# CogSP/CoEvoNet

Hardware: AMD Instinct MI355X
Metric: env-steps/sec (agent-steps of the whole job; generations/sec in gens_per_sec), Co-GA simple_adversary_v3 pop=200 HoF=5 (higher is better)
Workload: dtype f32

## Files before the change

### coevonet_amd/csrc/fc_forward.hip

```cpp
#include <cstdlib>

#include "coevo_common.hip.h"

namespace coevo {

#ifndef COEVO_HEAVY16_U
#define COEVO_HEAVY16_U 4
#endif
#ifndef COEVO_LIGHT_U
#define COEVO_LIGHT_U 8
#endif

typedef float f32x4_t __attribute__((ext_vector_type(4)));
__device__ inline float4 load_stream16(const float4 *p)
{
#ifdef COEVO_NO_NT
    return *p;
#else
    const f32x4_t v = __builtin_nontemporal_load(reinterpret_cast<const f32x4_t *>(p));
    return make_float4(v[0], v[1], v[2], v[3]);
#endif
}

template <int R, int P>
// ... 323 lines not shown
    if (row_wave && l < R * NACT) {
        const int r = l / NACT, o = l % NACT;
        float y = p_b3;
        const float4 *wr = reinterpret_cast<const float4 *>(&sm.w3s[pw][o][0]);
        const float4 *xr = reinterpret_cast<const float4 *>(&sm.h2[pw][r][0]);
#pragma unroll 8
        for (int k = 0; k < H2 / 4; ++k) {
            const float4 wv = wr[k], xv = xr[k];
            y = __builtin_fmaf(wv.x, xv.x, y);
            y = __builtin_fmaf(wv.y, xv.y, y);
            y = __builtin_fmaf(wv.z, xv.z, y);
            y = __builtin_fmaf(wv.w, xv.w, y);
        }
        sm.logit[pw][r][o] = y;
    }
    __syncthreads();
    COEVO_STAMP(5);

    if (row_wave && l < nrows[pw]) {
        int best = -1;
        float cur = -__builtin_inff();
#pragma unroll
        for (int o = 0; o < NACT; ++o) {
            const float v = sm.logit[pw][l][o];
            if (!__builtin_isfinite(v)) st |= COEVO_ST_BAD_OUT;
            if (v > cur) { cur = v; best = o; }
        }
        if (best < 0) { st |= COEVO_ST_NO_ACTION; best = 0; }
        const int row = row0[pw] + l;
        if constexpr (MODE >= MODE_FUSED) {
            a.act_cur[3 * a.row_game[row] + a.row_slot[row]] = best;
        } else {
            a.actions[row] = best;
        }
        if (a.logits) {
#pragma unroll
            for (int o = 0; o < NACT; ++o) a.logits[(size_t)row * COEVO_LOGIT_STRIDE + o] = sm.logit[pw][l][o];
        }
    }
    if (st) atomicOr(a.status, st);
    COEVO_STAMP(6);
}

template <int R>
struct FcSmemC {
    static constexpr int NG = (R + 3) / 4;
    static constexpr int RP = 4 * NG + 1;
    union {
        float par[13 * H1];
        float h1q[128][RP][4];
        float h1r[R][H1];
        struct { float h2[R][260]; float w3s[NACT][260]; } tail;
    };
    float xs0[4 * NG][COEVO_OBS_STRIDE];
    float red[4][16], red2[4][16];
    float logit[R][COEVO_LOGIT_STRIDE];
};

constexpr int FC2_MFMA = 0, FC2_DPP = 1;

#ifndef COEVO_SMALL_U
#define COEVO_SMALL_U 16
#endif

template <int J>
__device__ __forceinline__ void fmac_bcast(float &acc, float xv, float w)
{
    asm("v_fmac_f32_dpp %0, %1, %2 row_newbcast:%3 row_mask:0xf bank_mask:0xf" : "+v"(acc) : "v"(xv), "v"(w), "n"(J));
}

template <int R>
__device__ __forceinline__ void fmac_block16(float (&acc)[R], const float (&xv)[R], const float4 &p0, const float4 &p1,
                                             const float4 &p2, const float4 &p3)
{
#define COEVO_FMAC_K(J, W)                                   \
    _Pragma("unroll") for (int r = 0; r < R; ++r) fmac_bcast<J>(acc[r], xv[r], W);
    COEVO_FMAC_K(0, p0.x) COEVO_FMAC_K(1, p0.y) COEVO_FMAC_K(2, p0.z) COEVO_FMAC_K(3, p0.w)
    COEVO_FMAC_K(4, p1.x) COEVO_FMAC_K(5, p1.y) COEVO_FMAC_K(6, p1.z) COEVO_FMAC_K(7, p1.w)
    COEVO_FMAC_K(8, p2.x) COEVO_FMAC_K(9, p2.y) COEVO_FMAC_K(10, p2.z) COEVO_FMAC_K(11, p2.w)
    COEVO_FMAC_K(12, p3.x) COEVO_FMAC_K(13, p3.y) COEVO_FMAC_K(14, p3.z) COEVO_FMAC_K(15, p3.w)
#undef COEVO_FMAC_K
}

template <int R, int MODE, int FC2 = FC2_MFMA>
__device__ __forceinline__ void fc_policy_body_c(const FcArgs &a, FcSmemC<R> &sm, const coevo_fc_task *tasks, int first,
                                                 int n_tasks)
{
    static_assert((MODE == MODE_FUSED || MODE == MODE_OBS) && R * NACT <= 64 && R <= 8, "the lean merged cycle kernel");
    typedef float f32x4_acc __attribute__((ext_vector_type(4)));
    constexpr int NG = FcSmemC<R>::NG;
    COEVO_STAMP(0);
    const int t = threadIdx.x, w = t >> 6, l = t & 63;
    const bool active = first < n_tasks;
    const coevo_fc_task task = tasks[active ? first : n_tasks - 1];
    const int D = task.D, nrows = active ? task.n_rows : 0, row0 = task.row_begin;
    const float *net = a.slab + task.net_off;
    int st = 0;

    const int n_pieces = (D + 3) * (H1 / 4);
#pragma unroll
    for (int j = 0; j < 7; ++j)
        if (64 * w + 256 * j < n_pieces)
            __builtin_amdgcn_global_load_lds((const __attribute__((address_space(1))) void *)(net + 4 * (t + 256 * j)),
                                             (__attribute__((address_space(3))) void *)(&sm.par[4 * (64 * w + 256 * j)]),
                                             16, 0, 0);
    const float *b2p = net + fc_off_b2(D);
    float w3r[5];
    {
        const float *W3 = net + fc_off_w3(D);
#pragma unroll
        for (int j = 0; j < 5; ++j) w3r[j] = W3[t + 256 * j];
    }
    const float p_b2 = b2p[t], p_g2 = b2p[H2 + t], p_be2 = b2p[2 * H2 + t];
    const float p_b3 = (w == 0 && l < R * NACT) ? net[fc_off_b3(D) + l % NACT] : 0.0f;
    constexpr int US = COEVO_SMALL_U;
    static_assert(US % 4 == 0 && 128 % (2 * US) == 0, "buffers of whole 16-k blocks, consumed in pairs");
    const float4 *wps = reinterpret_cast<const float4 *>(net + fc_off_w2(D)) + (size_t)w * 128 * 64 + l;
    float4 sbufA[FC2 == FC2_DPP ? US : 1], sbufB[FC2 == FC2_DPP ? US : 1];

    if (w == 0 && l < 4 * NG) {
        float o[COEVO_OBS_STRIDE];
#pragma unroll
        for (int k = 0; k < COEVO_OBS_STRIDE; ++k) o[k] = 0.0f;
        if (l < nrows) {
            const int row = row0 + l;
            if constexpr (MODE == MODE_FUSED) {
                mpe_fused_observe(a.state, a.state_next, a.act_prev, a.game_limit, a.n_games, a.row_game[row],
                                  a.row_slot[row], a.cycle, a.pos_first, o);
            } else {
#pragma unroll
                for (int k = 0; k < 10; ++k) o[k] = (k < D) ? a.obs[(size_t)row * COEVO_OBS_STRIDE + k] : 0.0f;
            }
#pragma unroll
            for (int k = 0; k < 10; ++k)
                if (!__builtin_isfinite(o[k])) st |= COEVO_ST_BAD_INPUT;
        }
#pragma unroll
        for (int k = 0; k < COEVO_OBS_STRIDE; ++k) sm.xs0[l][k] = o[k];
    }
    COEVO_WSTAMP(0);
    __syncthreads();
    COEVO_WSTAMP(1);
    COEVO_CSTAMP(10);
    COEVO_STAMP(1);
    if constexpr (FC2 == FC2_DPP) {
#pragma unroll
        for (int uu = 0; uu < US; ++uu) sbufA[uu] = wps[(size_t)uu * 64];
#pragma unroll
        for (int uu = 0; uu < US; ++uu) sbufB[uu] = wps[(size_t)(US + uu) * 64];
    }

    const float *b1s = sm.par + D * H1;
    f32x4_acc c0[NG], c1[NG];
    {
        const float bia = b1s[t], bib = b1s[t + 256];
#pragma unroll
        for (int g = 0; g < NG; ++g)
#pragma unroll
            for (int i = 0; i < 4; ++i) { c0[g][i] = bia; c1[g][i] = bib; }
        float4 xk[NG][3];
#pragma unroll
        for (int g = 0; g < NG; ++g)
#pragma unroll
            for (int j = 0; j < 3; ++j) xk[g][j] = *reinterpret_cast<const float4 *>(&sm.xs0[4 * g + (l & 3)][4 * j]);
#pragma unroll
        for (int k = 0; k < 10; ++k) {
            if (k < D) {
                const float wa = sm.par[k * H1 + t], wb = sm.par[k * H1 + 256 + t];
#pragma unroll
                for (int g = 0; g < NG; ++g) {
// ... 4 lines not shown
                }
            }
        }
    }
    const float p_g1a = b1s[H1 + t], p_g1b = b1s[H1 + t + 256], p_be1a = b1s[2 * H1 + t], p_be1b = b1s[2 * H1 + t + 256];
    COEVO_STAMP(8);
    float v[2 * R];
#pragma unroll
    for (int r = 0; r < R; ++r) { v[2 * r] = c0[r >> 2][r & 3]; v[2 * r + 1] = c1[r >> 2][r & 3]; }
    {
        const float s = packed_totals<2 * R>(v, l);
        if (l < 2 * R) sm.red[w][l] = s;
    }
    COEVO_STAMP(9);
    COEVO_WSTAMP(2);
    __syncthreads();
    COEVO_WSTAMP(3);
    COEVO_STAMP(10);
    const int lr = l < R ? l : R - 1;
    {
        float tot = sm.red[0][2 * lr];
#pragma unroll
        for (int b = 1; b < 8; ++b) tot = tot + sm.red[b & 3][2 * lr + (b >> 2)];
        const float meanv = tot * (1.0f / H1);
#pragma unroll
        for (int r = 0; r < R; ++r) {
            const float m = __int_as_float(__builtin_amdgcn_readlane(__float_as_int(meanv), r));
            v[2 * r] = v[2 * r] - m;
            v[2 * r + 1] = v[2 * r + 1] - m;
        }
    }
    {
        float sq[2 * R];
#pragma unroll
        for (int j = 0; j < 2 * R; ++j) sq[j] = v[j] * v[j];
        const float s = packed_totals<2 * R>(sq, l);
        if (l < 2 * R) sm.red2[w][l] = s;
    }
    COEVO_WSTAMP(4);
    __syncthreads();
    COEVO_WSTAMP(5);
    {
        float tot = sm.red2[0][2 * lr];
#pragma unroll
        for (int b = 1; b < 8; ++b) tot = tot + sm.red2[b & 3][2 * lr + (b >> 2)];
        const float rstdv = 1.0f / __builtin_sqrtf(tot * (1.0f / H1) + LN_EPS);
        bool bad = false;
#pragma unroll
        for (int r = 0; r < R; ++r) {
            const float rstd = __int_as_float(__builtin_amdgcn_readlane(__float_as_int(rstdv), r));
            const float y0 = __builtin_fmaf(v[2 * r] * rstd, p_g1a, p_be1a);
            const float y1 = __builtin_fmaf(v[2 * r + 1] * rstd, p_g1b, p_be1b);
            if (r < nrows) bad = bad || bad_post_relu(y0) || bad_post_relu(y1);
            if constexpr (FC2 == FC2_DPP) {
                sm.h1r[r][t] = relu_keep_nan(y0);
                sm.h1r[r][t + 256] = relu_keep_nan(y1);
            } else {
                sm.h1q[t >> 2][r][t & 3] = relu_keep_nan(y0);
                sm.h1q[(t + 256) >> 2][r][t & 3] = relu_keep_nan(y1);
            }
        }
        if (bad) st |= COEVO_ST_BAD_FC1;
    }
    COEVO_WSTAMP(6);
    __syncthreads();
    COEVO_WSTAMP(7);
    COEVO_CSTAMP(11);
    COEVO_STAMP(2);

    f32x4_acc acc[NG];
    float u[R];
    if constexpr (FC2 == FC2_MFMA) {
#pragma unroll
    for (int g = 0; g < NG; ++g)
#pragma unroll
        for (int i = 0; i < 4; ++i) acc[g][i] = p_b2;
    {
        const float4 *wp = reinterpret_cast<const float4 *>(net + fc_off_w2(D)) + (size_t)w * 128 * 64 + l;
        constexpr int U = COEVO_LIGHT_U;
        static_assert(128 % (2 * U) == 0, "the k-quads are consumed in pairs of buffers");
        float4 bufA[U], bufB[U];
        auto issue = [&](float4 (&buf)[U], int kq) {
#pragma unroll
            for (int u = 0; u < U; ++u) buf[u] = load_stream16(wp + (size_t)(kq + u) * 64);
        };
        auto consume = [&](const float4 (&buf)[U], int kq) {
#pragma unroll
            for (int u = 0; u < U; ++u) {
                float4 x[NG];
#pragma unroll
                for (int g = 0; g < NG; ++g) x[g] = *reinterpret_cast<const float4 *>(&sm.h1q[kq + u][4 * g + (l & 3)][0]);
#pragma unroll
                for (int g = 0; g < NG; ++g) acc[g] = __builtin_amdgcn_mfma_f32_4x4x1f32(x[g].x, buf[u].x, acc[g], 0, 0, 0);
#pragma unroll
                for (int g = 0; g < NG; ++g) acc[g] = __builtin_amdgcn_mfma_f32_4x4x1f32(x[g].y, buf[u].y, acc[g], 0, 0, 0);
#pragma unroll
                for (int g = 0; g < NG; ++g) acc[g] = __builtin_amdgcn_mfma_f32_4x4x1f32(x[g].z, buf[u].z, acc[g], 0, 0, 0);
#pragma unroll
                for (int g = 0; g < NG; ++g) acc[g] = __builtin_amdgcn_mfma_f32_4x4x1f32(x[g].w, buf[u].w, acc[g], 0, 0, 0);
            }
        };
        issue(bufA, 0);
#pragma nounroll
        for (int kq = 0; kq < 128; kq += 2 * U) {
            issue(bufB, kq + U);
            __builtin_amdgcn_sched_barrier(0);
            consume(bufA, kq);
            if (kq + 2 * U < 128) issue(bufA, kq + 2 * U);
            __builtin_amdgcn_sched_barrier(0);
            consume(bufB, kq + U);
        }
    }
#pragma unroll
    for (int r = 0; r < R; ++r) u[r] = acc[r >> 2][r & 3];
    } else {
#pragma unroll
        for (int r = 0; r < R; ++r) u[r] = p_b2;
        const float *xrow = &sm.h1r[0][l & 15];
        auto issue_s = [&](float4 (&buf)[FC2 == FC2_DPP ? US : 1], int kq) {
#pragma unroll
            for (int uu = 0; uu < US; ++uu) buf[uu] = wps[(size_t)(kq + uu) * 64];
        };
        auto consume_s = [&](const float4 (&buf)[FC2 == FC2_DPP ? US : 1], int kq) {
#pragma unroll
            for (int b = 0; b < US / 4; ++b) {
                float xv[R];
#pragma unroll
                for (int r = 0; r < R; ++r) xv[r] = xrow[r * H1 + 4 * (kq + 4 * b)];
                fmac_block16<R>(u, xv, buf[4 * b], buf[4 * b + 1], buf[4 * b + 2], buf[4 * b + 3]);
            }
        };
#pragma nounroll
        for (int kq = 0; kq < 128; kq += 2 * US) {
            consume_s(sbufA, kq);
            if (kq + 2 * US < 128) issue_s(sbufA, kq + 2 * US);
            __builtin_amdgcn_sched_barrier(0);
            consume_s(sbufB, kq + US);
            if (kq + 3 * US < 128) issue_s(sbufB, kq + 3 * US);
            __builtin_amdgcn_sched_barrier(0);
        }
    }
    COEVO_STAMP(3);
    COEVO_WSTAMP(8);
    COEVO_CSTAMP(12);
    {
        const float s = packed_totals<R>(u, l);
        if (l < R) sm.red[w][l] = s;
    }
    __syncthreads();
    {
        const float tot = ((sm.red[0][lr] + sm.red[1][lr]) + sm.red[2][lr]) + sm.red[3][lr];
        const float meanv = tot * (1.0f / H2);
#pragma unroll
        for (int r = 0; r < R; ++r) u[r] = u[r] - __int_as_float(__builtin_amdgcn_readlane(__float_as_int(meanv), r));
        float sq[R];
#pragma unroll
        for (int r = 0; r < R; ++r) sq[r] = u[r] * u[r];
        const float s = packed_totals<R>(sq, l);
        if (l < R) sm.red2[w][l] = s;
    }
#pragma unroll
    for (int j = 0; j < 5; ++j) sm.tail.w3s[(t + 256 * j) >> 8][(t + 256 * j) & 255] = w3r[j];
    __syncthreads();
    {
        const float tot = ((sm.red2[0][lr] + sm.red2[1][lr]) + sm.red2[2][lr]) + sm.red2[3][lr];
        const float rstdv = 1.0f / __builtin_sqrtf(tot * (1.0f / H2) + LN_EPS);
        bool bad = false;
// ... 589 lines not shown
#pragma unroll
        for (int T = 0; T < 4; ++T) c2[T][i] = c2[T][i] - stat[i];
        const float s = (row16_tree_sum(c2[0][i] * c2[0][i]) + row16_tree_sum(c2[1][i] * c2[1][i])) +
                        (row16_tree_sum(c2[2][i] * c2[2][i]) + row16_tree_sum(c2[3][i] * c2[3][i]));
        if (lc == 0) sm.red[4 * lg + i][w] = s;
    }
    __syncthreads();
#pragma unroll
    for (int i = 0; i < 4; ++i) {
        const int row = 4 * lg + i;
        const float *rr = sm.red[row];
        const float tot = ((rr[0] + rr[1]) + rr[2]) + rr[3];
        const float rstd = 1.0f / __builtin_sqrtf(tot * (1.0f / H2) + LN_EPS);
#pragma unroll
        for (int T = 0; T < 4; ++T) {
            const float y = __builtin_fmaf(c2[T][i] * rstd, p_g2[T], p_be2[T]);
            if (row < nrows && bad_post_relu(y)) st |= COEVO_ST_BAD_FC2;
            sm.h2[row][64 * w + 16 * T + lc] = relu_keep_nan(y);
        }
    }
    asm volatile("" : "+v"(st));
    __syncthreads();
    COEVO_STAMP(4);

    if (t < 16 * NACT) {
        const int r = t / NACT, o = t % NACT;
        float y = p_b3;
        const float4 *wr = reinterpret_cast<const float4 *>(&sm.w3s[o][0]);
        const float4 *xr = reinterpret_cast<const float4 *>(&sm.h2[r][0]);
#pragma unroll 8
        for (int k = 0; k < H2 / 4; ++k) {
            const float4 wv = wr[k], xv = xr[k];
            y = __builtin_fmaf(wv.x, xv.x, y);
            y = __builtin_fmaf(wv.y, xv.y, y);
            y = __builtin_fmaf(wv.z, xv.z, y);
            y = __builtin_fmaf(wv.w, xv.w, y);
        }
        sm.logit[r][o] = y;
    }
    __syncthreads();
    COEVO_STAMP(5);
    if (t < nrows) {
        int best = -1;
        float cur = -__builtin_inff();
#pragma unroll
        for (int o = 0; o < NACT; ++o) {
            const float v = sm.logit[t][o];
            if (!__builtin_isfinite(v)) st |= COEVO_ST_BAD_OUT;
            if (v > cur) { cur = v; best = o; }
        }
        if (best < 0) { st |= COEVO_ST_NO_ACTION; best = 0; }
        if constexpr (MODE >= MODE_FUSED) {
            const int row = row0 + t;
            a.act_cur[3 * a.row_game[row] + a.row_slot[row]] = best;
        } else {
            a.actions[row0 + t] = best;
        }
        if (a.logits) {
#pragma unroll
            for (int o = 0; o < NACT; ++o) a.logits[(size_t)(row0 + t) * COEVO_LOGIT_STRIDE + o] = sm.logit[t][o];
        }
    }
    if (st) atomicOr(a.status, st);
    COEVO_STAMP(6);
}

template <int R, int MODE = MODE_FUSED>
__global__ __launch_bounds__(256, 4) void fc_cycle16_kernel(FcArgs a)
{
    __shared__ __attribute__((aligned(16))) union Cycle16Smem {
        FcMfma16Smem heavy;
#if COEVO_COMPACT
        FcSmemC<R> light;
#else
        FcSmem<R, 1> light;
#endif
    } sm;
    static_assert(sizeof(sm) <= 40960, "four workgroups per CU");
    stamp_begin(a.stamps);
    if ((int)blockIdx.x < a.n_heavy)
        fc_policy_mfma16_body<MODE>(a, sm.heavy, a.tasks[blockIdx.x]);
    else
#if COEVO_COMPACT
        fc_policy_body_c<R, MODE>(a, sm.light, a.light_tasks, (int)blockIdx.x - a.n_heavy, a.n_light);
#else
        fc_policy_body<R, MODE, 1>(a, sm.light, a.light_tasks, (int)blockIdx.x - a.n_heavy, a.n_light);
#endif
    stamp_end(a.stamps);
}

template <int R, int MODE = MODE_FUSED>
__global__ __launch_bounds__(256, 2) void fc_cycle_small_kernel(FcArgs a)
{
    __shared__ __attribute__((aligned(16))) FcSmemC<R> sm;
    stamp_begin(a.stamps);
    const bool heavy = (int)blockIdx.x < a.n_heavy;
    fc_policy_body_c<R, MODE, FC2_DPP>(a, sm, heavy ? a.tasks : a.light_tasks, heavy ? (int)blockIdx.x : (int)blockIdx.x - a.n_heavy,
                                       heavy ? a.n_heavy : a.n_light);
    stamp_end(a.stamps);
}

template <int R>
struct FcSmemP {
    static constexpr int NG = (R + 3) / 4;
    float par[13 * H1];
    float h1r[R][H1];
    float h2[R][260];
    float w3s[NACT][260];
    float xs0[4 * NG][COEVO_OBS_STRIDE];
    float red[4][16], red2[4][16];
    float logit[R][COEVO_LOGIT_STRIDE];
    double gs[8][24];
    float p2[3][H2];
    float pb3[8];
    int rowinfo[8][4];
    int ctl[4];
};

#ifndef COEVO_SYNC_SPINS
#define COEVO_SYNC_SPINS (1 << 21)
#endif

struct PersistArgs {
    int n_cycles;
    int32_t *sync;
    double *state_alt;
    int32_t *act_plain;
    double *rewards;
    coevo_final_pack pack;
};

__global__ void sync_clear_kernel(int32_t *w, int n)
{
    const int i = blockIdx.x * blockDim.x + threadIdx.x;
    if (i < n) w[i] = 0;
}

template <int R>
__global__ __launch_bounds__(256, 2) void fc_rollout_small_kernel(FcArgs a, PersistArgs pa)
{
    __shared__ __attribute__((aligned(16))) FcSmemP<R> sm;
    static_assert(sizeof(FcSmemP<R>) <= 80 * 1024, "two workgroups per CU");
    constexpr int NG = FcSmemP<R>::NG;
    constexpr int US = COEVO_SMALL_U;
    typedef float f32x4_acc __attribute__((ext_vector_type(4)));
    const int t = threadIdx.x, w = t >> 6, l = t & 63;
    const bool heavy = (int)blockIdx.x < a.n_heavy;
    const coevo_fc_task task = heavy ? a.tasks[blockIdx.x] : a.light_tasks[(int)blockIdx.x - a.n_heavy];
    const int D = task.D, nrows = task.n_rows, row0 = task.row_begin;
    const float *net = a.slab + task.net_off;
    const size_t N = (size_t)a.n_games;
    int st = 0;

    const int n_pieces = (D + 3) * (H1 / 4);
#pragma unroll
    for (int j = 0; j < 7; ++j)
        if (64 * w + 256 * j < n_pieces)
            __builtin_amdgcn_global_load_lds((const __attribute__((address_space(1))) void *)(net + 4 * (t + 256 * j)),
                                             (__attribute__((address_space(3))) void *)(&sm.par[4 * (64 * w + 256 * j)]),
                                             16, 0, 0);
    {
        const float *W3 = net + fc_off_w3(D);
#pragma unroll
        for (int j = 0; j < 5; ++j) sm.w3s[(t + 256 * j) >> 8][(t + 256 * j) & 255] = W3[t + 256 * j];
    }
    {
        const float *b2p = net + fc_off_b2(D);
// ... 608 lines not shown
```

### coevonet_amd/genetic_algorithm.py

```python
from __future__ import annotations

import os
import time

import numpy as np
import torch

from . import lib as L
from .fcnetwork import FCNetwork
from .game_logic import create_agent
from .mpe.simple_adversary import ENV_SEED
from .rollout import DeviceRollout, HostEnvRollout, RolloutPlan, effective_steps

ROLES = ("agent_0", "agent_1", "adversary_0")
ROLE_D = {"agent_0": 10, "agent_1": 10, "adversary_0": 8}
ROLE_SLOT = {"agent_0": 1, "agent_1": 2, "adversary_0": 0}
RET_SLOT = {"agent_0": 0, "agent_1": 1, "adversary_0": 2}
SIGMA_ATTR = {"agent_0": "mutation_power_agent_0", "agent_1": "mutation_power_agent_1",
              "adversary_0": "mutation_power_adversary"}
N_EVAL = 10


def evaluate_current_weights(agent_0, agent_1, adversary, env, args):
    from .game_logic import play_game
    tot = [0.0, 0.0, 0.0]
    for _ in range(N_EVAL):
        r = play_game(env=env, player1=agent_0.model, player2=agent_1.model, adversary=adversary.model, args=args, eval=True)
        for s in range(3):
            tot[s] += r[s]
    return tot[0] / 10, tot[1] / 10, tot[2] / 10


def mutate_elites(env, elites, args, role):
    sigma = {"agent_0": args.mutation_power_agent_0, "agent_1": args.mutation_power_agent_1}.get(
        role, args.mutation_power_adversary)
    children = []
    for i in range(args.population - 1):
        child = elites[i % args.elites_number].clone(env, args, role)
        child.mutate(sigma)
        children.append(child)
    return children


def adapt_mutation_power(args, gen, hist):
    def worse(h):
        return gen > 10 and np.mean(h[-10:]) < np.mean(h[-20:-10])
    if worse(hist["agent_0"]):
        args.mutation_power_agent_0 = min(args.mutation_power_agent_1 * 1.2, args.max_mutation_power)
    else:
        args.mutation_power_agent_0 = max(args.mutation_power_agent_0 * 0.95, args.min_mutation_power)
    if worse(hist["agent_1"]):
        args.mutation_power_agent_1 = min(args.mutation_power_agent_1 * 1.2, args.max_mutation_power)
    else:
        args.mutation_power_agent_1 = max(args.mutation_power_agent_1 * 0.95, args.min_mutation_power)
    if worse(hist["adversary_0"]):
        args.mutation_power_adversary = min(args.mutation_power_adversary * 1.2, args.max_mutation_power)
    else:
        args.mutation_power_adversary = max(args.mutation_power_adversary * 0.95, args.min_mutation_power)


def small_shard_rows(n_local, hof, cus, pop):
    if n_local >= pop or not 1 <= hof <= 8:
        return 16
    per_cu = 2 if os.environ.get("COEVO_PERSISTENT", "1") != "0" else 1
    if 3 * n_local + 6 * hof * -(-n_local // hof) <= per_cu * cus:
        return hof
    return 16


def cohort_partition(n_local, K):
    bounds = np.array([k * n_local // K for k in range(K + 1)], dtype=np.int64)
    return bounds, np.searchsorted(bounds[1:], np.arange(n_local), side="right").astype(np.int32)


DEFAULT_COHORTS = 1
DEVICE_LOOP_COHORTS = 2
SMALL_SHARD = 80


class GAEngine:

    def __init__(self, pop, hof, elites, limit_train=None, limit_eval=None, max_cycles=25, device="cuda",
                 env_seed=ENV_SEED, rng="device_philox", philox_seed=0, env="device", first_ordinal=1,
                 shard=(0, 1), gather=None, timing_pairs=4096, cohorts=1, gather_packed=None):
        assert 1 <= elites <= pop and hof >= 1
        self.pop, self.hof, self.E = pop, hof, elites
        self.rng_mode, self.philox_seed, self.env_mode = rng, int(philox_seed), env
        self.device = device
        self.rank, self.world = shard
        self.gather = gather
        self.gather_packed = gather_packed
        if self.world > 1 and pop % self.world:
            raise ValueError(f"population {pop} is not divisible by the number of ranks {self.world}")
        self.lo = self.rank * pop // self.world
        self.hi = (self.rank + 1) * pop // self.world
        self.n_local = self.hi - self.lo
        self.T_train = effective_steps(limit_train, max_cycles)
        self.T_eval = effective_steps(limit_eval, max_cycles)
        self.n_cycles = (max(self.T_train, self.T_eval) + 2) // 3
        self.first_ordinal = first_ordinal
        self.env_seed = env_seed
        self.stride = {r: L.fc_slab_stride(ROLE_D[r]) for r in ROLES}
        self.P = {r: L.fc_param_count(ROLE_D[r]) for r in ROLES}
        self.base, off = {}, 0
        for r in ROLES:
            self.base[r] = {}
            for region, count in (("pop", pop), ("hof", hof), ("elite", elites), ("stale", 1), ("hof_tmp", hof),
                                  ("elite_prev", elites)):
                self.base[r][region] = off
                off += count * self.stride[r]
        self.slab = torch.zeros(off, dtype=torch.float32, device=device)
        net_off, net_D, ids = [], [], {}

        def net(region, role, i):
            key = (region, role, i)
            if key not in ids:
                ids[key] = len(net_off)
                net_off.append(self.base[role][region] + i * self.stride[role])
                net_D.append(ROLE_D[role])
            return ids[key]

        games = []
        h = hof
        for role in ROLES:
            for i in range(self.lo, self.hi):
                for k in range(h):
                    if role == "agent_0":
                        a0, a1, adv = net("pop", role, i), net("hof", "agent_1", h - 1 - k), net("hof", "adversary_0", h - 1 - k)
                    elif role == "agent_1":
                        a0, a1, adv = net("hof", "agent_0", h - 1 - k), net("pop", role, i), net("hof", "adversary_0", h - 1 - k)
                    else:
                        a0, a1, adv = net("hof", "agent_0", h - 1 - k), net("hof", "agent_0", h - 1 - k), net("pop", role, i)
                    games.append((adv, a0, a1))
        self.n_main = len(games)
        for _ in range(N_EVAL):
            games.append((net("hof", "adversary_0", h - 1), net("hof", "agent_0", h - 1), net("hof", "agent_1", h - 1)))
        heavy_rows = int(os.environ.get("COEVO_HEAVY_ROWS", "0"))
        if heavy_rows <= 0:
            cus = torch.cuda.get_device_properties(device).multi_processor_count if (env == "device" and str(device) != "cpu") else 0
            heavy_rows = small_shard_rows(self.n_local, hof, cus, pop) if (cus and cohorts <= 1) else 16
        host_k = int(os.environ.get("COEVO_HOST_COHORTS", "0")) or max(1, min(4, len(games) // 700))
        self.K = max(1, min(int(cohorts) if env == "device" else host_k, self.n_local))
        row_order = "class" if env == "device" else "cohort"
        self._set_cohort_bounds()
        game_cohort = None
        if self.K > 1:
            per_ind = np.repeat(cohort_partition(self.n_local, self.K)[1], self.hof)
            game_cohort = np.concatenate([per_ind, per_ind, per_ind, np.full(N_EVAL, self.K - 1)]).astype(np.int32)
        try:
            self.plan = RolloutPlan(np.array(games), net_off, net_D, device=device, heavy_rows=heavy_rows,
                                    n_cohorts=self.K, game_cohort=game_cohort, row_order=row_order)
        except ValueError:
            self.K = 1
            self._set_cohort_bounds()
            self.plan = RolloutPlan(np.array(games), net_off, net_D, device=device, heavy_rows=heavy_rows,
                                    row_order=row_order)
        if env == "device":
            self.ro = DeviceRollout(self.plan, self.slab, env_seed=env_seed, timing_pairs=timing_pairs)
        else:
            self.ro = HostEnvRollout(self.plan, self.slab, env_seed=env_seed)
        f32 = dict(dtype=torch.float32, device=device)
        self.dist_all = torch.zeros(3, pop, **f32)
        self.dist = {r: self.dist_all[i] for i, r in enumerate(ROLES)}
        self.div = {r: torch.zeros(1, **f32) for r in ROLES}
        self.fitness = {r: torch.zeros(pop, **f32) for r in ROLES}
        self.order = {r: torch.zeros(pop, dtype=torch.int32, device=device) for r in ROLES}
        self.sigma = {r: torch.zeros(1, **f32) for r in ROLES}
        self.sigma_prev = {r: torch.zeros(1, **f32) for r in ROLES}
        self.last_reward = torch.zeros(3, pop, 3, dtype=torch.float64, device=device)
        self.pack_local = torch.zeros(3, self.n_local, 4, dtype=torch.float64, device=device)
        self.pack_all = torch.zeros(self.world, 3, self.n_local, 4, dtype=torch.float64, device=device)
        self.parent_idx = torch.tensor([c % elites for c in range(max(pop - 1, 1))], dtype=torch.int32, device=device)
        self.hof_shift_idx = torch.arange(1, max(hof, 2), dtype=torch.int32, device=device)
        self.iota = torch.arange(max(hof, elites, 2), dtype=torch.int32, device=device)
        self.generation = 0
        self.steps_per_generation = 3 * pop * hof * self.T_train + N_EVAL * self.T_eval

    def _ptr(self, role, region, i=0):
        return self.slab.data_ptr() + 4 * (self.base[role][region] + i * self.stride[role])

    def upload(self, role, region, first, flat_np):
        flat = torch.from_numpy(np.ascontiguousarray(flat_np, dtype=np.float32)).to(self.device)
        L.call("coevo_fc_pack", L._p(flat), self._ptr(role, region, first), flat.shape[0], ROLE_D[role])
        if region in ("pop", "stale"):
            self._dist_current = False
        return flat

    def download(self, role, region, first, n):
        if region == "pop":
            self.flush_breeding()
        out = torch.zeros(n, self.P[role], dtype=torch.float32, device=self.device)
        L.call("coevo_fc_unpack", self._ptr(role, region, first), L._p(out), n, ROLE_D[role])
        return out.cpu().numpy()

    def load_initial(self, pop_flat, hof_flat):
        keep = []
        for r in ROLES:
            keep.append(self.upload(r, "pop", 0, pop_flat[r]))
            keep.append(self.upload(r, "hof", 0, hof_flat[r]))
            keep.append(self.upload(r, "stale", 0, pop_flat[r][self.pop - 1:self.pop]))
        torch.cuda.current_stream().synchronize()

    def _ordinal_base(self, gen):
        return self.first_ordinal + gen * (3 * self.pop * self.hof + N_EVAL)

    def rollout(self, gen, with_prev_eval):
        ro, M = self.ro, 3 * self.pop * self.hof
        limits = np.zeros(self.plan.n_games, dtype=np.int32)
        limits[:self.n_main] = self.T_train
        if with_prev_eval:
            limits[self.n_main:] = self.T_eval
        ro.set_limits(limits)
        base = self._ordinal_base(gen)
        per_phase = self.n_local * self.hof
        if self.env_mode == "device":
            for ph in range(3):
                ro.reset(ph * per_phase, per_phase, base + ph * self.pop * self.hof + self.lo * self.hof)
            if with_prev_eval:
                ro.reset(self.n_main, N_EVAL, self._ordinal_base(gen - 1) + M)
        else:
            ords = np.zeros(self.plan.n_games, dtype=np.int64)
            for ph in range(3):
                ords[ph * per_phase:(ph + 1) * per_phase] = (base + ph * self.pop * self.hof + self.lo * self.hof
                                                             + np.arange(per_phase))
            ords[self.n_main:] = (self._ordinal_base(gen - 1) + M + np.arange(N_EVAL)) if with_prev_eval else 0
            ro.reset_from_ordinals(ords)
        ro.run(self.n_cycles)

    def eval_only(self, gen):
        ro, M = self.ro, 3 * self.pop * self.hof
        limits = np.zeros(self.plan.n_games, dtype=np.int32)
        limits[self.n_main:] = self.T_eval
        ro.set_limits(limits)
        if self.env_mode == "device":
            ro.reset(0, self.n_main, 0)
            ro.reset(self.n_main, N_EVAL, self._ordinal_base(gen) + M)
        else:
            ords = np.zeros(self.plan.n_games, dtype=np.int64)
            ords[self.n_main:] = self._ordinal_base(gen) + M + np.arange(N_EVAL)
# ... 708 lines not shown
```

### coevonet_amd/lib.py

```python
from __future__ import annotations

import ctypes as C
import os

import numpy as np
import torch

HERE = os.path.dirname(os.path.abspath(__file__))
LIB_PATH = os.environ.get("COEVO_LIB") or os.path.join(HERE, "libcoevo.so")

OBS_STRIDE = 12
LOGIT_STRIDE = 8
FC_MAX_ROWS = 32
MPE_STATE_DOUBLES = 24
STAMP_SLOTS = 32
ST_NAMES = {1: "input contains inf or NaN", 2: "output contains inf or NaN after fc1",
            4: "output contains inf or NaN after fc2", 8: "output contains inf or NaN",
            16: "no action selected (current_best_position = -1)",
            32: "persistent rollout: a workgroup timed out waiting for the other rows of its games (COEVO_ST_SYNC_TIMEOUT)",
            64: "fp16 forward: a task with a bad width, row count or unaligned net offset was skipped (COEVO_ST_BAD_TASK)"}

DQN_LOGIT_STRIDE = 32
DQN_FC1_TILED = 0x100
DQN_MAX_ROWS = 16
DQN_TASK_DTYPE = np.dtype([("net_off", "<i8"), ("row_begin", "<i4"), ("n_rows", "<i4")])

TASK_DTYPE = np.dtype([("net_off", "<i8"), ("row_begin", "<i4"), ("n_rows", "<i4"), ("D", "<i4"),
                       ("reserved", "<i4")])


class PCG64State(C.Structure):
    _fields_ = [("state_hi", C.c_uint64), ("state_lo", C.c_uint64), ("inc_hi", C.c_uint64), ("inc_lo", C.c_uint64)]

    @classmethod
    def from_seed(cls, seed):
        st = np.random.PCG64(seed).state["state"]
        m = (1 << 64) - 1
        return cls(st["state"] >> 64, st["state"] & m, st["inc"] >> 64, st["inc"] & m)


class PerturbJob(C.Structure):
    _fields_ = [("parent_slab", C.c_void_p), ("parent_idx", C.c_void_p), ("child_slab", C.c_void_p),
                ("sigma_dev", C.c_void_p), ("dist_ref", C.c_void_p), ("dist_partial", C.c_void_p),
                ("child_first", C.c_int32), ("n_children", C.c_int32), ("D", C.c_int32),
                ("stream_lo_first", C.c_uint32), ("stream_hi", C.c_uint32), ("pad", C.c_int32)]


class FinalizeJob(C.Structure):
    _fields_ = [("dist_partial", C.c_void_p), ("dist", C.c_void_p), ("head", C.c_void_p), ("n_blocks", C.c_int32),
                ("n", C.c_int32), ("first", C.c_int32), ("pad", C.c_int32)]


class ResetSeg(C.Structure):
    _fields_ = [("game_first", C.c_int32), ("count", C.c_int32), ("first_ordinal", C.c_uint64)]


class FinalPack(C.Structure):
    _fields_ = [("out", C.c_void_p), ("dist", C.c_void_p), ("n_roles", C.c_int32), ("n_local", C.c_int32), ("hof", C.c_int32),
                ("dist_pitch", C.c_int32), ("dist_first", C.c_int32), ("reserved", C.c_int32)]


class RolloutDesc(C.Structure):
    _fields_ = [("slab", C.c_void_p), ("heavy", C.c_void_p), ("n_heavy", C.c_int32), ("heavy_max_rows", C.c_int32),
                ("light", C.c_void_p), ("n_light", C.c_int32), ("light_max_rows", C.c_int32),
                ("state", C.c_void_p), ("n_games", C.c_int32), ("n_cycles", C.c_int32),
                ("row_game", C.c_void_p), ("row_slot", C.c_void_p), ("game_rows", C.c_void_p),
                ("actions", C.c_void_p), ("status", C.c_void_p), ("game_limit", C.c_void_p),
                ("rewards", C.c_void_p), ("pos_first", C.c_int32), ("n_cohorts", C.c_int32),
                ("state_alt", C.c_void_p), ("actions_by_game", C.c_void_p), ("light_stamps", C.c_void_p),
                ("heavy_begin", C.c_void_p), ("light_begin", C.c_void_p),
                ("merged", C.c_int32), ("concurrent_hint", C.c_int32), ("stamps_armed", C.c_int32), ("sync_cleared", C.c_int32),
                ("sync_words", C.c_void_p), ("pack", C.c_void_p)]


class HostCohort(C.Structure):
    _fields_ = [("heavy", C.c_void_p), ("light", C.c_void_p), ("games", C.c_void_p), ("n_heavy", C.c_int32),
                ("heavy_max_rows", C.c_int32), ("n_light", C.c_int32), ("light_max_rows", C.c_int32),
                ("n_games", C.c_int32), ("row_first", C.c_int32), ("n_rows", C.c_int32), ("reserved", C.c_int32)]


class HostRolloutDesc(C.Structure):
    _fields_ = [("slab", C.c_void_p), ("state", C.c_void_p), ("game_rows", C.c_void_p), ("game_limit", C.c_void_p),
                ("obs_host", C.c_void_p), ("obs_dev", C.c_void_p), ("actions_host", C.c_void_p),
                ("actions_dev", C.c_void_p), ("status", C.c_void_p), ("cohorts", C.c_void_p), ("phase_us", C.c_void_p),
                ("n_games", C.c_int32), ("n_rows", C.c_int32), ("n_cycles", C.c_int32), ("n_cohorts", C.c_int32),
                ("pos_first", C.c_int32), ("zero_copy", C.c_int32), ("reset_ordinals", C.c_void_p),
                ("reset_rng", PCG64State)]


class FrameCohort(C.Structure):
    _fields_ = [("tasks", C.c_void_p * 2), ("rows", C.c_void_p * 2), ("frames_host", C.c_void_p),
                ("frames_dev", C.c_void_p), ("actions_host", C.c_void_p), ("actions_dev", C.c_void_p),
                ("workspace", C.c_void_p), ("n_tasks", C.c_int32 * 2), ("max_rows", C.c_int32 * 2),
                ("game_first", C.c_int32), ("n_games", C.c_int32)]


class FramesRolloutDesc(C.Structure):
    _fields_ = [("slab", C.c_void_p), ("status", C.c_void_p), ("game_state", C.c_void_p), ("acc", C.c_void_p),
                ("game_ordinal0", C.c_void_p), ("limit", C.c_void_p), ("cohorts", C.c_void_p), ("phase_us", C.c_void_p),
                ("generation", C.c_int64), ("ordinals_per_gen", C.c_int64), ("seed", C.c_uint64),
                ("n_games", C.c_int32), ("n_cohorts", C.c_int32), ("C", C.c_int32), ("n_actions", C.c_int32),
                ("T", C.c_int32), ("reserved", C.c_int32)]


class GaSelectRole(C.Structure):
    _fields_ = [("dist", C.c_void_p), ("rewards", C.c_void_p), ("diversity", C.c_void_p), ("fitness", C.c_void_p),
                ("order", C.c_void_p), ("best_dist", C.c_void_p), ("game_first", C.c_int32), ("slot", C.c_int32)]


class GaAdaptArgs(C.Structure):
    _fields_ = [("rewards", C.c_void_p), ("gen_dev", C.c_void_p), ("hist", C.c_void_p), ("sig_hist", C.c_void_p),
# ... 261 lines not shown
```

### coevonet_amd/rollout.py

```python
from __future__ import annotations

import ctypes as _ct

import os

import numpy as np
import torch

from . import lib as L
from .mpe import simple_adversary as sa

LIGHT_ROWS = 8
HEAVY_ROWS = 32


class RolloutPlan:

    def __init__(self, game_nets, net_off, net_D, device="cuda", heavy_rows=HEAVY_ROWS, n_cohorts=1,
                 game_cohort=None, split_rows=None, row_order="class"):
        game_nets = np.asarray(game_nets, dtype=np.int64)
        self.n_games = int(game_nets.shape[0])
        by_net = {}
        for g in range(self.n_games):
            for slot in range(3):
                by_net.setdefault(int(game_nets[g, slot]), []).append((g, slot))
        for net, rows in by_net.items():
            d = int(net_D[net])
            for g, slot in rows:
                assert d == (8 if slot == 0 else 10), "net width does not match the env slot it plays"
        if game_cohort is not None:
            cohort = np.asarray(game_cohort, dtype=np.int32)
            assert cohort.shape == (self.n_games,) and cohort.min() >= 0
            for net, rows in by_net.items():
                if len(rows) <= LIGHT_ROWS and len({int(cohort[g]) for g, _ in rows}) != 1:
                    raise ValueError("a net with few rows (one task) plays in two cohorts: this partition is not valid")
            if len(np.unique(cohort)) != int(cohort.max()) + 1:
                raise ValueError("empty cohort")
        else:
            cohort = self._assign_cohorts(by_net, self.n_games, max(1, int(n_cohorts)))
        self.n_cohorts = int(cohort.max()) + 1 if self.n_games else 1
        self.game_cohort_np = cohort
        light = [[] for _ in range(self.n_cohorts)]
        heavy = [[] for _ in range(self.n_cohorts)]
        for net, rows in by_net.items():
            if split_rows is not None:
                assert self.n_cohorts == 1 and 1 <= split_rows <= LIGHT_ROWS
                for i in range(0, len(rows), split_rows):
                    light[0].append((net, rows[i:i + split_rows]))
            elif len(rows) <= LIGHT_ROWS:
                light[int(cohort[rows[0][0]])].append((net, rows))
            else:
                for k in range(self.n_cohorts):
                    mine = [(g, slot) for g, slot in rows if cohort[g] == k]
                    for i in range(0, len(mine), heavy_rows):
                        heavy[k].append((net, mine[i:i + heavy_rows]))
        heavy = [self._xcd_order(h) for h in heavy]
        self.heavy_begin_np = np.cumsum([0] + [len(h) for h in heavy]).astype(np.int32)
        self.light_begin_np = np.cumsum([0] + [len(x) for x in light]).astype(np.int32)
        assert row_order in ("class", "cohort")
        row_game, row_slot = [], []
        tasks = {"heavy": [[] for _ in range(self.n_cohorts)], "light": [[] for _ in range(self.n_cohorts)]}
        cohort_rows = np.zeros(self.n_cohorts + 1, dtype=np.int64)

        def number(name, k):
            for net, rows in (heavy if name == "heavy" else light)[k]:
                tasks[name][k].append((int(net_off[net]), len(row_game), len(rows), int(net_D[net]), 0))
                for g, slot in rows:
                    row_game.append(g)
                    row_slot.append(slot)

        if row_order == "class":
            for name in ("heavy", "light"):
                for k in range(self.n_cohorts):
                    number(name, k)
            self.cohort_row_begin_np = None
        else:
            for k in range(self.n_cohorts):
                number("heavy", k)
                number("light", k)
                cohort_rows[k + 1] = len(row_game)
            self.cohort_row_begin_np = cohort_rows
        tasks = {name: [t for per in tasks[name] for t in per] for name in tasks}
        self.n_rows = len(row_game)
        assert self.n_rows == 3 * self.n_games
        game_rows = np.zeros((self.n_games, 3), dtype=np.int32)
        for r, (g, slot) in enumerate(zip(row_game, row_slot)):
            game_rows[g, slot] = r
        self.row_game_np = np.asarray(row_game, dtype=np.int32)
        self.row_slot_np = np.asarray(row_slot, dtype=np.int32)
        self.game_rows_np = game_rows
        self.heavy_np = np.array(tasks["heavy"], dtype=L.TASK_DTYPE) if tasks["heavy"] else np.zeros(0, L.TASK_DTYPE)
        self.light_np = np.array(tasks["light"], dtype=L.TASK_DTYPE) if tasks["light"] else np.zeros(0, L.TASK_DTYPE)
        self.heavy_max = int(max([t[2] for t in tasks["heavy"]], default=0))
        self.light_max = int(max([t[2] for t in tasks["light"]], default=0))
        self.device = device
        if device is not None:
            self.row_game = torch.from_numpy(self.row_game_np).to(device)
            self.row_slot = torch.from_numpy(self.row_slot_np).to(device)
            self.game_rows = torch.from_numpy(game_rows.reshape(-1).copy()).to(device)
            self.heavy = L.tasks_to_device(self.heavy_np, device) if len(self.heavy_np) else None
            self.light = L.tasks_to_device(self.light_np, device) if len(self.light_np) else None

    @staticmethod
    def _assign_cohorts(by_net, n_games, n_cohorts):
        cohort = np.zeros(n_games, dtype=np.int32)
        if n_cohorts <= 1 or n_games == 0:
            return cohort
        parent = list(range(n_games))

        def find(x):
            while parent[x] != x:
                parent[x] = parent[parent[x]]
                x = parent[x]
            return x

        for rows in by_net.values():
            if len(rows) <= LIGHT_ROWS:
                r0 = find(rows[0][0])
                for g, _ in rows[1:]:
                    parent[find(g)] = r0
        comps = {}
        for g in range(n_games):
            comps.setdefault(find(g), []).append(g)
        for c, games in enumerate(sorted(comps.values(), key=lambda c: c[0])):
            cohort[games] = c % n_cohorts
        used = np.unique(cohort)
        remap = {int(u): i for i, u in enumerate(used)}
        return np.array([remap[int(c)] for c in cohort], dtype=np.int32)

    @staticmethod
    def _xcd_order(heavy):
        if len(heavy) < 16:
            return heavy
        by_net = sorted(heavy, key=lambda t: t[0])
        n = len(by_net)
        buckets = [by_net[b * n // 8:(b + 1) * n // 8] for b in range(8)]
        out = []
        for q in range(max(len(b) for b in buckets)):
            for x in range(8):
                if q < len(buckets[x]):
                    out.append(buckets[x][q])
        return out

    def distinct_weight_bytes_per_cycle(self):
        seen = {}
        for arr in (self.heavy_np, self.light_np):
            for t in arr:
                seen[int(t["net_off"])] = L.fc_param_count(int(t["D"])) * 4
        return sum(seen.values())
# ... 393 lines not shown
```

### include/coevo.h

```cpp
#ifndef COEVO_H
#define COEVO_H

#include <stddef.h>
#include <stdint.h>

#ifdef __cplusplus
extern "C" {
#endif

#define COEVO_VERSION 103

#define COEVO_OK 0
#define COEVO_ERR_ARG (-1)
#define COEVO_ERR_HIP (-2)
#define COEVO_ERR_UNSUPPORTED (-3)

#define COEVO_ST_BAD_INPUT 1
#define COEVO_ST_BAD_FC1 2
#define COEVO_ST_BAD_FC2 4
#define COEVO_ST_BAD_OUT 8
#define COEVO_ST_NO_ACTION 16
#define COEVO_ST_SYNC_TIMEOUT 32
#define COEVO_ST_BAD_TASK 64

#define COEVO_FC_H1 512
#define COEVO_FC_H2 256
#define COEVO_FC_NACT 5
#define COEVO_OBS_STRIDE 12
#define COEVO_LOGIT_STRIDE 8
#define COEVO_FC_MAX_ROWS 32
#define COEVO_STAMP_SLOTS 32

#define COEVO_SLOT_ADVERSARY 0
#define COEVO_SLOT_AGENT_0 1
#define COEVO_SLOT_AGENT_1 2

int coevo_version(void);
const char *coevo_build_flags(void);

int64_t coevo_fc_param_count(int D);
int64_t coevo_fc_slab_stride(int D);
int coevo_fc_pack(const float *flat, float *slab, int n, int D, void *stream);
int coevo_fc_unpack(const float *slab, float *flat, int n, int D, void *stream);

typedef struct {
    int64_t net_off;
    int32_t row_begin;
    int32_t n_rows;
    int32_t D;
    int32_t reserved;
} coevo_fc_task;

int coevo_fc_forward_argmax(const float *slab, const coevo_fc_task *tasks, int n_tasks, int max_rows_per_task,
                            const float *obs, int32_t *actions, float *logits, int32_t *status, void *stream);
int coevo_fc_forward_merged(const float *slab, const coevo_fc_task *heavy_tasks, int n_heavy, int heavy_max_rows,
                            const coevo_fc_task *light_tasks, int n_light, int light_max_rows, const float *obs,
                            int32_t *actions, float *logits, int32_t *status, void *stream);

int64_t coevo_fc16_slab_stride(int D);
int coevo_fc16_pack(const float *flat, void *slab, int n, int D, void *stream);
int coevo_fc16_unpack(const void *slab, float *flat, int n, int D, void *stream);
int coevo_fc16_forward_argmax(const void *slab, const coevo_fc_task *tasks, int n_tasks, int max_rows_per_task,
                              const float *obs, int32_t *actions, float *logits, int32_t *status, void *stream);

#define COEVO_MPE_STATE_DOUBLES 24
typedef struct {
    uint64_t pcg_state_hi, pcg_state_lo, pcg_inc_hi, pcg_inc_lo;
} coevo_pcg64;

int coevo_mpe_reset(double *state, int n_games, int game_first, int count, coevo_pcg64 rng, uint64_t first_ordinal,
                    void *stream);
typedef struct { int32_t game_first, count; uint64_t first_ordinal; } coevo_reset_seg;
int coevo_mpe_reset_multi(double *state, int n_games, const coevo_reset_seg *segs , int n_segs,
                          coevo_pcg64 rng, void *stream);
int coevo_mpe_reset_multi_arm(double *state, int n_games, const coevo_reset_seg *segs , int n_segs,
                              coevo_pcg64 rng, uint64_t *stamps, int n_stamps, void *stream);
int coevo_mpe_reset_multi_prep(double *state, int n_games, const coevo_reset_seg *segs , int n_segs,
                               coevo_pcg64 rng, uint64_t *stamps, int n_stamps, int32_t *zero_words, int n_zero, void *stream);
int coevo_mpe_reset_gen(double *state, int n_games, int game_first, int count, coevo_pcg64 rng, int64_t first_ordinal,
                        const int32_t *gen_dev, int64_t ordinals_per_gen, void *stream);
int coevo_mpe_observe(const double *state, int n_games, const int32_t *row_game, const int32_t *row_slot,
                      int n_rows, float *obs, void *stream);
int coevo_mpe_step(double *state, int n_games, const int32_t *game_rows, const int32_t *actions, int cycle,
                   const int32_t *game_limit, int pos_first, void *stream);
int coevo_mpe_host_reset(double *state, int n_games, coevo_pcg64 rng, const int64_t *ordinals );
int coevo_mpe_host_reset_games(double *state, int n_games, coevo_pcg64 rng, const int64_t *ordinals ,
                               const int32_t *games, int lo, int hi );
int coevo_mpe_host_observe(const double *state, int n_games, const int32_t *row_game, const int32_t *row_slot,
                           int n_rows, float *obs);
int coevo_mpe_host_step(double *state, int n_games, const int32_t *game_rows, const int32_t *actions, int n_rows,
                        int cycle, const int32_t *game_limit, int pos_first);
int coevo_mpe_host_step_games(double *state, int n_games, const int32_t *game_rows, const int32_t *actions, int cycle,
                              const int32_t *game_limit, int pos_first, const int32_t *games, int lo, int hi, int observe,
                              float *obs);

typedef struct {
    const coevo_fc_task *heavy;
    const coevo_fc_task *light;
    const int32_t *games;
    int32_t n_heavy, heavy_max_rows, n_light, light_max_rows;
    int32_t n_games;
    int32_t row_first, n_rows;
    int32_t reserved;
} coevo_host_cohort;
typedef struct {
    const float *slab;
    double *state;
    const int32_t *game_rows;
    const int32_t *game_limit;
    float *obs_host;
    float *obs_dev;
    int32_t *actions_host;
    int32_t *actions_dev;
    int32_t *status;
    const coevo_host_cohort *cohorts;
    double *phase_us;
    int32_t n_games, n_rows, n_cycles, n_cohorts, pos_first;
    int32_t zero_copy;
    const int64_t *reset_ordinals;
    coevo_pcg64 reset_rng;
} coevo_host_rollout_desc;
void *coevo_host_rollout_create(int n_threads, int n_cohorts);
void coevo_host_rollout_destroy(void *ctx);
int coevo_host_rollout_threads(void *ctx);
int coevo_mpe_host_rollout(void *ctx, const coevo_host_rollout_desc *desc, void *stream);
#define COEVO_PLACE_ON_NODE 1
#define COEVO_PLACE_ONE_L3 2
#define COEVO_PLACE_NODE_UNKNOWN 4
#define COEVO_PLACE_SHORT 8
int coevo_host_placement_choose(const char *allowed, const char *node_cpus, const char *l3_groups, const char *smt_groups,
                                int caller_cpu, int n_threads, int ctx_index, int32_t *cpus_out, int32_t *flags_out);
int coevo_host_rollout_placement(void *ctx, int32_t *cpus_out, int max_cpus, int32_t *info_out);
void *coevo_host_rollout_alloc(void *ctx, size_t bytes);
int coevo_host_rollout_debug_seed_counters(void *ctx, uint32_t value);
// ... 265 lines not shown
```

Measured before the change: 133.2 million.

## Keep a budgeted prefix of light-task weights cache-resident via plain loads

Adds a per-task RESIDENT flag, set on the host for a prefix of each cohort's population networks that fits a configurable byte budget (default 224 MB, sized against the MI355X last-level cache). For flagged light tasks the fused cycle kernel loads FC2 weights with ordinary loads instead of nontemporal streaming loads, so those networks can stay in cache across steps. Unflagged tasks keep streaming so they do not evict the resident set. The risk is cache thrashing if the budget is wrong, and an extra branch plus a second template instantiation in the kernel.

```diff
diff --git a/coevonet_amd/csrc/fc_forward.hip b/coevonet_amd/csrc/fc_forward.hip
--- a/coevonet_amd/csrc/fc_forward.hip
+++ b/coevonet_amd/csrc/fc_forward.hip
@@ -429,10 +429,11 @@
 #undef COEVO_FMAC_K
 }
 
-template <int R, int MODE, int FC2 = FC2_MFMA>
+template <int R, int MODE, int FC2 = FC2_MFMA, bool RES = false>
 __device__ __forceinline__ void fc_policy_body_c(const FcArgs &a, FcSmemC<R> &sm, const coevo_fc_task *tasks, int first,
                                                  int n_tasks)
 {
+    static_assert(!RES || FC2 == FC2_MFMA, "the vector-ALU form streams with plain loads already");
     static_assert((MODE == MODE_FUSED || MODE == MODE_OBS) && R * NACT <= 64 && R <= 8, "the lean merged cycle kernel");
     typedef float f32x4_acc __attribute__((ext_vector_type(4)));
     constexpr int NG = FcSmemC<R>::NG;
@@ -603,7 +604,7 @@
         float4 bufA[U], bufB[U];
         auto issue = [&](float4 (&buf)[U], int kq) {
 #pragma unroll
-            for (int u = 0; u < U; ++u) buf[u] = load_stream16(wp + (size_t)(kq + u) * 64);
+            for (int u = 0; u < U; ++u) buf[u] = RES ? wp[(size_t)(kq + u) * 64] : load_stream16(wp + (size_t)(kq + u) * 64);
         };
         auto consume = [&](const float4 (&buf)[U], int kq) {
 #pragma unroll
@@ -1359,7 +1360,13 @@
         fc_policy_mfma16_body<MODE>(a, sm.heavy, a.tasks[blockIdx.x]);
     else
 #if COEVO_COMPACT
-        fc_policy_body_c<R, MODE>(a, sm.light, a.light_tasks, (int)blockIdx.x - a.n_heavy, a.n_light);
+    {
+        const int li = (int)blockIdx.x - a.n_heavy;
+        if (MODE == MODE_FUSED && li < a.n_light && (a.light_tasks[li].reserved & COEVO_TASK_RESIDENT))
+            fc_policy_body_c<R, MODE, FC2_MFMA, MODE == MODE_FUSED>(a, sm.light, a.light_tasks, li, a.n_light);
+        else
+            fc_policy_body_c<R, MODE>(a, sm.light, a.light_tasks, li, a.n_light);
+    }
 #else
         fc_policy_body<R, MODE, 1>(a, sm.light, a.light_tasks, (int)blockIdx.x - a.n_heavy, a.n_light);
 #endif
diff --git a/coevonet_amd/genetic_algorithm.py b/coevonet_amd/genetic_algorithm.py
--- a/coevonet_amd/genetic_algorithm.py
+++ b/coevonet_amd/genetic_algorithm.py
@@ -71,6 +71,31 @@
 def cohort_partition(n_local, K):
     bounds = np.array([k * n_local // K for k in range(K + 1)], dtype=np.int64)
     return bounds, np.searchsorted(bounds[1:], np.arange(n_local), side="right").astype(np.int32)
+
+
+RESIDENT_MB_DEFAULT = 224
+
+
+def resident_budget_bytes():
+    v = os.environ.get("COEVO_RESIDENT_MB", "").strip().lower()
+    if v == "all":
+        return float("inf")
+    return (float(v) if v else RESIDENT_MB_DEFAULT) * 1e6
+
+
+def resident_enabled(env, heavy_rows, n_local, pop):
+    return env == "device" and heavy_rows == 16 and n_local >= pop
+
+
+def resident_prefix(budget_bytes, fixed_bytes, individual_bytes, bounds):
+    K = len(bounds) - 1
+    sizes = np.diff(np.asarray(bounds, dtype=np.int64))
+    left = budget_bytes - fixed_bytes
+    if left <= 0 or K <= 0:
+        return np.zeros(K, dtype=np.int64)
+    if left == float("inf"):
+        return sizes
+    return np.minimum(sizes, int(left // (K * individual_bytes)))
 
 
 DEFAULT_COHORTS = 1
@@ -147,14 +172,25 @@
         if self.K > 1:
             per_ind = np.repeat(cohort_partition(self.n_local, self.K)[1], self.hof)
             game_cohort = np.concatenate([per_ind, per_ind, per_ind, np.full(N_EVAL, self.K - 1)]).astype(np.int32)
+        resident = resident_enabled(env, heavy_rows, self.n_local, pop)
+
+        def resident_nets():
+            if not resident:
+                return ()
+            ind_bytes = sum(4 * self.stride[r] for r in ROLES)
+            n = resident_prefix(resident_budget_bytes(), (hof + elites + 1) * ind_bytes, ind_bytes, self.cohort_bounds)
+            return [ids[("pop", r, self.lo + i)] for r in ROLES for k in range(self.K)
+                    for i in range(int(self.cohort_bounds[k]), int(self.cohort_bounds[k]) + int(n[k]))]
+
         try:
             self.plan = RolloutPlan(np.array(games), net_off, net_D, device=device, heavy_rows=heavy_rows,
-                                    n_cohorts=self.K, game_cohort=game_cohort, row_order=row_order)
+                                    n_cohorts=self.K, game_cohort=game_cohort, row_order=row_order,
+                                    resident_nets=resident_nets())
         except ValueError:
             self.K = 1
             self._set_cohort_bounds()
             self.plan = RolloutPlan(np.array(games), net_off, net_D, device=device, heavy_rows=heavy_rows,
-                                    row_order=row_order)
+                                    row_order=row_order, resident_nets=resident_nets())
         if env == "device":
             self.ro = DeviceRollout(self.plan, self.slab, env_seed=env_seed, timing_pairs=timing_pairs)
         else:
diff --git a/coevonet_amd/lib.py b/coevonet_amd/lib.py
--- a/coevonet_amd/lib.py
+++ b/coevonet_amd/lib.py
@@ -27,6 +27,7 @@
 
 TASK_DTYPE = np.dtype([("net_off", "<i8"), ("row_begin", "<i4"), ("n_rows", "<i4"), ("D", "<i4"),
                        ("reserved", "<i4")])
+TASK_RESIDENT = 1
 
 
 class PCG64State(C.Structure):
diff --git a/coevonet_amd/rollout.py b/coevonet_amd/rollout.py
--- a/coevonet_amd/rollout.py
+++ b/coevonet_amd/rollout.py
@@ -17,7 +17,7 @@
 class RolloutPlan:
 
     def __init__(self, game_nets, net_off, net_D, device="cuda", heavy_rows=HEAVY_ROWS, n_cohorts=1,
-                 game_cohort=None, split_rows=None, row_order="class"):
+                 game_cohort=None, split_rows=None, row_order="class", resident_nets=()):
         game_nets = np.asarray(game_nets, dtype=np.int64)
         self.n_games = int(game_nets.shape[0])
         by_net = {}
@@ -62,9 +62,12 @@
         tasks = {"heavy": [[] for _ in range(self.n_cohorts)], "light": [[] for _ in range(self.n_cohorts)]}
         cohort_rows = np.zeros(self.n_cohorts + 1, dtype=np.int64)
 
+        resident_nets = frozenset(int(n) for n in resident_nets)
+
         def number(name, k):
             for net, rows in (heavy if name == "heavy" else light)[k]:
-                tasks[name][k].append((int(net_off[net]), len(row_game), len(rows), int(net_D[net]), 0))
+                flags = L.TASK_RESIDENT if (name == "light" and net in resident_nets) else 0
+                tasks[name][k].append((int(net_off[net]), len(row_game), len(rows), int(net_D[net]), flags))
                 for g, slot in rows:
                     row_game.append(g)
                     row_slot.append(slot)
diff --git a/include/coevo.h b/include/coevo.h
--- a/include/coevo.h
+++ b/include/coevo.h
@@ -50,6 +50,7 @@
     int32_t D;
     int32_t reserved;
 } coevo_fc_task;
+#define COEVO_TASK_RESIDENT 1
 
 int coevo_fc_forward_argmax(const float *slab, const coevo_fc_task *tasks, int n_tasks, int max_rows_per_task,
                             const float *obs, int32_t *actions, float *logits, int32_t *status, void *stream);
```

New measurement: 149.8 million (median of 6 runs). 12.5% higher.
